# heli-sudoo/HKD-MPC

Measured on NVIDIA B200. Metric: batched HS-DDP solves/sec, higher is better.
Workload: dtype f64

## Files before the change

hkd-mpc_b200/csrc/hsddp_device.cuh:

```cuda
#pragma once
#include <cuda_runtime.h>
#include <stdint.h>
#include <cstddef>
#include "../../include/hsddp_b200.h"
#include "hkd_model.cuh"

#ifdef HSDDP_PROFILE
#define PROF_DECL long long prof_t0_ = clock64();
#define PROF_MARK(sm, slot)                                                         \
    do {                                                                            \
        if (threadIdx.x == 0) {                                                     \
            const long long t1_ = clock64();                                        \
            (sm).profacc[slot] += (unsigned long long)(t1_ - prof_t0_);             \
            prof_t0_ = t1_;                                                         \
        }                                                                           \
    } while (0)
#else
#define PROF_DECL
#define PROF_MARK(sm, slot) do { } while (0)
#endif

namespace hsddp {

constexpr int kThreads = 128;
// ... 30 lines not shown
    unsigned nmask[MAXPH];
    long long ref_off;
    double dt;
    unsigned char ph_of_stage[HSDDP_MAX_STAGES];
    unsigned char ph_of_node[HSDDP_MAX_STAGES + MAXPH];
    unsigned char ss_size[MAXPH];
    unsigned char tdmask[2][MAXPH];
};
static_assert(sizeof(DevSchedule) % 4 == 0, "bind_problem copies the schedule word by word");

struct SolverState {
    double actual_cost, merit, feas, dV_1, dV_2;
    double max_tconstr_prev, max_pconstr_prev, max_tconstr, max_pconstr, merit_rho;
    double reg;
    int rollout_ok, sweep_ok;
};

struct SolveCtl {
    int iter, iter_ou, iter_in, n_sweeps, n_trials, status;
    int active;
    int have_trial;
    int max_al, max_ddp;
    double cost0, feas0;
    double trial_cost, trial_feas;
};

struct BatchPtrs {
    int n_problems, max_stages, max_nodes, _pad;
    const DevSchedule* sched;
    const int* sched_id;
    const double *xr, *ur, *prel, *xinit;
    double* x0;
    double *Xbar, *X, *Xsim_t, *Defect, *dX;
    double *Ubar, *U, *U_t, *dU;
    double* KdX;
    double* K;
    double* lq;
    double* tq;
    double* gcon;
    double* reb;
    double* hcon;
    double* al;
    double* g0h0;
    SolverState* state;
    SolveCtl* ctl;
    const int* active;
    const int* n_active;
    int* next_active;
    int* next_count;
    int* zero_count;
    int sweep_w1_min;
    int lr_external;
    int _pad2;
    double *ls_X, *ls_Defect, *ls_Xsim, *ls_U, *ls_Ut, *ls_gcon, *ls_hcon, *ls_res;
    int* ls_mail;
    const int* order;
    const int* budget;
    hsddp_info* info;
    hsddp_iter_record* trace;
    unsigned long long* counters;
    int* work_counter;
    int* sm_slots;
    hsddp_constraint_params cp;
};

struct Smem;
struct __align__(16) Smem {
    double H[ro(24)], Y[ro(24)];
    double Z[zo(24)];
    double Qux[ro(16) + kQuuPad];
    double Quu[ro(12)];
    double rec[2][LQ_STRIDE];
    double dfc2[2][24];
    double G[24], Gn[24], Qx[24], Qu[24], wu[24], vtmp[24], vtmp2[24];
    double lxxd[24], lxxTd[24], lxxw[12], lxxTw[12];
    double swdt[4];
    double swc[16];
    double red[kThreads];
    DevSchedule sc;
    SolverState st;
    SolveCtl ctl;
    hsddp_constraint_params cp;
    hsddp_options opt;
    double *Xbar, *X, *Xsim_t, *Defect, *dX, *Ubar, *U, *U_t, *dU, *KdX, *K, *lqg, *tq, *gcon, *reb, *hcon, *al, *g0h0;
    const double *xr, *ur, *prel, *xinit, *x0;
    unsigned long long* prof;
    unsigned long long profacc[16];
    int pid;
    int rot;
    int flag;
    int ibuf[4];
    double dbuf[8];
};

static_assert(offsetof(Smem, dfc2) - offsetof(Smem, H) == sizeof(double) * kSweepDoubles, "kSweepDoubles must cover H..rec");
static_assert(32 * 113 <= kSweepDoubles, "LQ staging buffer does not fit");

__device__ __forceinline__ int virtual_tid(const Smem& sm);
__device__ inline void assign_rotation(int* sm_slots, int& rot_out) {
    unsigned smid;
    asm volatile("mov.u32 %0, %%smid;" : "=r"(smid));
    rot_out = atomicAdd(&sm_slots[smid & 255], 1) & 3;
}
__device__ __forceinline__ int virtual_tid(const Smem& sm) { return (int)((threadIdx.x + 32u * (unsigned)sm.rot) & (kThreads - 1)); }

__device__ __forceinline__ double warp_sum(double v) {
// ... 672 lines not shown
```

hkd-mpc_b200/csrc/hsddp_kernels.cu:

```cuda
#include <cuda_runtime.h>
#include <cooperative_groups.h>
#include <cstdio>
#include <cstdlib>
#include <cstring>
#include <string>
#include <vector>
#include <map>
#include <algorithm>
#include "hsddp_device.cuh"
#include "hsddp_sweep.cuh"
#include "hsddp_sweep_w1.cuh"
#include "hsddp_lr_w1.cuh"

#ifndef HSDDP_MIN_BLOCKS
#define HSDDP_MIN_BLOCKS 6
#endif

namespace hsddp {

constexpr int hsddp_batch_max_groups = 16;

__device__ inline void prepare_merit_block(Smem& sm) {
    if (threadIdx.x == 0) {
        SolverState& st = sm.st;
// ... 355 lines not shown
        if (threadIdx.x == 0) for (int i = 0; i < 16; ++i) atomicAdd(&sm.prof[i], sm.profacc[i]);
#endif
    }
}

struct ResumeLists {
    const int* list[hsddp_batch_max_groups];
    const int* count[hsddp_batch_max_groups];
    int n;
};
template <int MINB>
__global__ void __launch_bounds__(kThreads, MINB) k_solve_resume(BatchPtrs bp, hsddp_options opt, ResumeLists rl) {
    __shared__ Smem sm;
    if (threadIdx.x == 0) assign_rotation(bp.sm_slots, sm.rot);
    for (;;) {
        __syncthreads();
        if (threadIdx.x == 0) {
            int q = atomicAdd(bp.work_counter, 1), pid = -1;
            for (int g = 0; g < rl.n; ++g) {
                const int c = *rl.count[g];
                if (q < c) { pid = rl.list[g][q]; break; }
                q -= c;
            }
            sm.ibuf[3] = pid;
        }
        __syncthreads();
        const int pid = sm.ibuf[3];
        if (pid < 0) break;
        bind_problem(sm, bp, pid);
        if (threadIdx.x == 0) sm.opt = opt;
        __syncthreads();
        while (sm.ctl.active) {
            iter_prep_block(sm, bp);
            iter_sweep_block(sm, bp);
            if (!sm.ctl.active) break;
            iter_forward_block(sm, bp);
        }
        solve_finish_block(sm, bp);
        if (threadIdx.x == 0) { bp.state[pid] = sm.st; bp.ctl[pid] = sm.ctl; }
    }
}

enum SolvePhase { PH_BEGIN = 0, PH_PREP, PH_SWEEP, PH_FORWARD };
#ifndef HSDDP_MINB_SWEEP
#define HSDDP_MINB_SWEEP 5
#endif
#ifndef HSDDP_MINB_OTHER
#define HSDDP_MINB_OTHER 6
#endif
template <int PH>
__global__ void __launch_bounds__(kThreads, PH == 2 ? HSDDP_MINB_SWEEP : HSDDP_MINB_OTHER) k_phase(BatchPtrs bp, hsddp_options opt) {
    __shared__ Smem sm;
    if (PH == PH_PREP && bp.zero_count && blockIdx.x == 0 && threadIdx.x == 0) *bp.zero_count = 0;
    if (bp.n_active && (int)blockIdx.x >= *bp.n_active) return;
    if (PH == PH_SWEEP && bp.n_active && bp.sweep_w1_min > 0 && *bp.n_active >= bp.sweep_w1_min) return;
    const int pid = bp.active ? bp.active[blockIdx.x] : (int)blockIdx.x;
    if (threadIdx.x == 0) assign_rotation(bp.sm_slots, sm.rot);
    bind_problem(sm, bp, pid);
    if (threadIdx.x == 0) sm.opt = opt;
    __syncthreads();
#ifdef HSDDP_PROFILE
    if (threadIdx.x == 0) for (int i = 0; i < 16; ++i) sm.profacc[i] = 0;
    __syncthreads();
#endif
    if (PH == PH_BEGIN) solve_begin_block(sm, bp);
    if (PH == PH_PREP) iter_prep_block(sm, bp);
    if (PH == PH_SWEEP) iter_sweep_block(sm, bp);
    if (PH == PH_FORWARD) {
        if (sm.ctl.active) iter_forward_block(sm, bp);
    }
    __syncthreads();
    if (PH == PH_BEGIN || PH == PH_FORWARD) {
        if (sm.ctl.active) {
            if (threadIdx.x == 0) bp.next_active[atomicAdd(bp.next_count, 1)] = pid;
        } else {
            solve_finish_block(sm, bp);
        }
    }
    if (threadIdx.x == 0) { bp.state[pid] = sm.st; bp.ctl[pid] = sm.ctl; }
#ifdef HSDDP_PROFILE
    if (threadIdx.x == 0) for (int i = 0; i < 16; ++i) atomicAdd(&sm.prof[i], sm.profacc[i]);
#endif
}

enum StepOp { OP_RESET = 0, OP_ROLLOUT, OP_COST, OP_LQ, OP_SWEEP, OP_SWEEP_REG, OP_LINEAR, OP_MERIT, OP_FORWARD, OP_NOMINAL, OP_AL, OP_REB };

__global__ void __launch_bounds__(kThreads, HSDDP_MIN_BLOCKS) k_step(BatchPtrs bp, hsddp_options opt, int op, double arg, double* darg, int* ok) {
    __shared__ Smem sm;
    const int pid = blockIdx.x;
    if (threadIdx.x == 0) assign_rotation(bp.sm_slots, sm.rot);
    bind_problem(sm, bp, pid);
    if (threadIdx.x == 0) sm.opt = opt;
    __syncthreads();
    int okv = 1;
    switch (op) {
        case OP_RESET: cold_start_block(sm); break;
        case OP_ROLLOUT: okv = hybrid_rollout_block<false>(sm, arg) ? 1 : 0; break;
        case OP_COST: compute_cost_block(sm); break;
        case OP_LQ: lq_approximation_block(sm); break;
        case OP_SWEEP: okv = backward_sweep_block(sm, arg) ? 1 : 0; break;
        case OP_SWEEP_REG: {
            if (threadIdx.x == 0) sm.st.reg = darg[pid];
            __syncthreads();
            int nsw;
            okv = backward_sweep_regularized_block(sm, nsw) ? 1 : 0;
            if (threadIdx.x == 0) darg[pid] = sm.st.reg;
        } break;
        case OP_LINEAR: linear_rollout_block(sm, arg); break;
        case OP_MERIT: prepare_merit_block(sm); break;
        case OP_FORWARD: {
            const double cost_prev = sm.st.actual_cost, merit_prev = sm.st.merit;
            double eps_acc; int ntr;
            okv = line_search_block<false>(sm, eps_acc, ntr) ? 1 : 0;
            if (!okv) { __syncthreads(); if (threadIdx.x == 0) { sm.st.actual_cost = cost_prev; sm.st.merit = merit_prev; } }
            if (threadIdx.x == 0 && darg) darg[pid] = eps_acc;
        } break;
        case OP_NOMINAL: update_nominal_block(sm); break;
        case OP_AL: update_al_block(sm); break;
        case OP_REB: update_reb_block(sm); break;
        default: break;
    }
    __syncthreads();
    if (threadIdx.x == 0) { bp.state[pid] = sm.st; if (ok) ok[pid] = okv; }
}

__global__ void k_command(BatchPtrs bp, int n_steps, hsddp_mpc_command* out) {
    const int pid = blockIdx.x;
    const DevSchedule& sc = bp.sched[bp.sched_id[pid]];
    hsddp_mpc_command& cmd = out[pid];
    __shared__ int s_stage[HSDDP_CMD_MAX_STEPS], s_node[HSDDP_CMD_MAX_STEPS], s_phase[HSDDP_CMD_MAX_STEPS];
    if (threadIdx.x == 0) {
        int s = 0, i = 0;
        for (int k = 0; k < n_steps; ++k) {
            if (s >= sc.horizon[i]) { s = 0; i++; }
            if (i >= sc.n_phases) { i = sc.n_phases - 1; s = sc.horizon[i] - 1; }
// ... 428 lines not shown
}

}

using namespace hsddp;

static thread_local std::string g_last_error;
const char* hsddp_last_error(void) { return g_last_error.c_str(); }
namespace hsddp { void set_last_error(const std::string& s) { g_last_error = s; } }

#define CK(call)                                                                                   \
    do {                                                                                           \
        cudaError_t e_ = (call);                                                                   \
        if (e_ != cudaSuccess) {                                                                   \
            g_last_error = std::string(#call) + ": " + cudaGetErrorString(e_);                     \
            return HSDDP_ERR_CUDA;                                                                 \
        }                                                                                          \
    } while (0)

struct hsddp_batch {
    int device = 0;
    cudaStream_t stream = nullptr;
    cudaEvent_t ev0 = nullptr, ev1 = nullptr;
    cudaEvent_t slots[8] = {nullptr, nullptr, nullptr, nullptr, nullptr, nullptr, nullptr, nullptr};
    unsigned long long n_solve_launches = 0, n_step_launches = 0;
    int n_sm = 0, blocks_per_sm = 1;
    BatchPtrs bp{};
    std::vector<void*> allocs;
    std::vector<DevSchedule> h_sched;
    std::vector<int> h_sched_id;
    bool has_problems = false;
    bool cold = true;
    float last_ms = 0.f;
    int* d_ok = nullptr;
    double* d_darg = nullptr;
    int solve_mode = 0;
    int* d_active[2] = {nullptr, nullptr};
    int* d_count = nullptr;
    int last_rounds = 0;
    int sweep_kind = 2;
    int w1_min_blocks = 1036;
    bool lr_w1 = true;
    int* d_order = nullptr;
    bool have_order = false, use_order = true;
    bool cluster_ls = true;
    static constexpr int kClusterLsMax = 32;
    static constexpr int kMaxGroups = 16;
    int phased_min_group = 1024;
    int hybrid_rounds = 20, hybrid_groups = 4, hybrid_min_group = 256;
    int phased_groups = 4;
    cudaStream_t gstream[kMaxGroups] = {};
    cudaEvent_t gevent[kMaxGroups] = {};
    cudaEvent_t ev_fork = nullptr;
    hsddp_mpc_command* d_cmd = nullptr;
    bool mpc_ready = false;
    GaitLib lib{};
    int *d_sched_gait = nullptr, *d_sched_window = nullptr, *d_mpc_err = nullptr;
    MpcSched* d_mpc = nullptr;
    float plan = 0.f;
    int node_stride = 0, n_sched = 0;
    bool h_sched_stale = false;
    cudaEvent_t ev_u0 = nullptr, ev_u1 = nullptr;
    int n_gaits = 0;
    std::vector<int> slot_refs;
    std::vector<int> slot_free;
    int* d_restart = nullptr;
    double* d_restart_x0 = nullptr;
    size_t d_restart_cap = 0, d_restart_x0_cap = 0;
    int* d_budget = nullptr;
    long long budget_rounds = -1;
    bool slots_marked = false;
};

namespace {

template <class F>
int guarded(F&& body) {
    try {
        return body();
    } catch (const std::bad_alloc&) {
        g_last_error = "out of host memory";
        return HSDDP_ERR_ARG;
    } catch (const std::exception& e) {
        g_last_error = std::string("unexpected exception: ") + e.what();
        return HSDDP_ERR_STATE;
    } catch (...) {
        g_last_error = "unexpected exception";
        return HSDDP_ERR_STATE;
    }
}

template <class T>
int dalloc(hsddp_batch* b, T** p, size_t n) {
    void* q = nullptr;
    CK(cudaMalloc(&q, n * sizeof(T)));
    b->allocs.push_back(q);
    *p = (T*)q;
    return HSDDP_OK;
}

template <class T>
int scratch(hsddp_batch* b, T** p, size_t* cap, size_t n) {
    if (*cap >= n) return HSDDP_OK;
    void* q = nullptr;
    CK(cudaMalloc(&q, n * sizeof(T)));
    if (*p) {
// ... 48 lines not shown
    else bad = check_budget(opt->max_AL_iter, opt->max_DDP_iter);
    if (bad) { g_last_error = std::string("invalid hsddp_options: ") + bad; return HSDDP_ERR_ARG; }
    return HSDDP_OK;
}

int launch_step(hsddp_batch* b, const hsddp_options* opt, int op, double arg, double* darg_dev, int32_t* ok_host, bool sync = true) {
    if (!b || !b->has_problems) { g_last_error = "no problems set"; return HSDDP_ERR_STATE; }
    int rc = check_opt(opt);
    if (rc) return rc;
    CK(cudaSetDevice(b->device));
    const hsddp_options o = opt ? *opt : default_options();
    k_step<<<b->bp.n_problems, kThreads, 0, b->stream>>>(b->bp, o, op, arg, darg_dev, b->d_ok);
    CK(cudaGetLastError());
    b->n_step_launches++;
    if (ok_host) CK(cudaMemcpyAsync(ok_host, b->d_ok, sizeof(int) * b->bp.n_problems, cudaMemcpyDeviceToHost, b->stream));
    if (sync || ok_host) CK(cudaStreamSynchronize(b->stream));
    if (op != OP_RESET) b->cold = false;
    return HSDDP_OK;
}

}

extern "C" {

static int batch_init(hsddp_batch* b, int device) {
    CK(cudaSetDevice(device));
    b->device = device;
    CK(cudaStreamCreateWithFlags(&b->stream, cudaStreamNonBlocking));
    CK(cudaEventCreate(&b->ev0));
    CK(cudaEventCreate(&b->ev1));
    CK(cudaEventCreate(&b->ev_u0));
    CK(cudaEventCreate(&b->ev_u1));
    for (int i = 0; i < 8; ++i) CK(cudaEventCreate(&b->slots[i]));
    cudaDeviceProp prop;
    CK(cudaGetDeviceProperties(&prop, device));
    b->n_sm = prop.multiProcessorCount;
    CK(cudaOccupancyMaxActiveBlocksPerMultiprocessor(&b->blocks_per_sm, k_solve, kThreads, 0));
    if (b->blocks_per_sm < 1) b->blocks_per_sm = 1;
    if (const char* e = getenv("HSDDP_BLOCKS_PER_SM")) {
        const int v = atoi(e);
        if (v >= 1 && v <= b->blocks_per_sm) b->blocks_per_sm = v;
    }
    CK(cudaEventCreateWithFlags(&b->ev_fork, cudaEventDisableTiming));
    if (const char* e = getenv("HSDDP_PHASED_GROUPS")) {
        const int v = atoi(e);
        if (v >= 1 && v <= hsddp_batch::kMaxGroups) b->phased_groups = v;
    }
    if (const char* e = getenv("HSDDP_PHASED_MIN_GROUP")) { const int v = atoi(e); if (v >= 1) b->phased_min_group = v; }
    if (const char* e = getenv("HSDDP_HYBRID_ROUNDS")) b->hybrid_rounds = atoi(e);
    if (const char* e = getenv("HSDDP_HYBRID_GROUPS")) { const int v = atoi(e); if (v >= 1 && v <= hsddp_batch::kMaxGroups) b->hybrid_groups = v; }
    if (const char* e = getenv("HSDDP_SWEEP_KIND")) b->sweep_kind = atoi(e);
    CK(cudaFuncSetAttribute(k_sweep_w1, cudaFuncAttributePreferredSharedMemoryCarveout, cudaSharedmemCarveoutMaxShared));
    CK(cudaFuncSetAttribute(k_lr_w1, cudaFuncAttributePreferredSharedMemoryCarveout, cudaSharedmemCarveoutMaxShared));
    if (const char* e = getenv("HSDDP_W1_MIN_BLOCKS")) b->w1_min_blocks = atoi(e);
    if (const char* e = getenv("HSDDP_LR_W1")) b->lr_w1 = atoi(e) != 0;
    if (const char* e = getenv("HSDDP_QUEUE_ORDER")) b->use_order = atoi(e) != 0;
    if (const char* e = getenv("HSDDP_CLUSTER_LS")) b->cluster_ls = atoi(e) != 0;
    if (const char* e = getenv("HSDDP_SOLVE_MODE")) {
        const int v = atoi(e);
        if (v >= 0 && v <= 3) b->solve_mode = v;
    }
    return HSDDP_OK;
}

int hsddp_batch_create(int device, hsddp_batch** out) {
    if (!out) return HSDDP_ERR_ARG;
    *out = nullptr;
    int n = 0;
    CK(cudaGetDeviceCount(&n));
    if (device < 0 || device >= n) { g_last_error = "no such CUDA device (this library has no CPU fallback)"; return HSDDP_ERR_CUDA; }
    return guarded([&]() -> int {
        hsddp_batch* b = new hsddp_batch();
        const int rc = batch_init(b, device);
        if (rc != HSDDP_OK) { hsddp_batch_destroy(b); return rc; }
        *out = b;
        return HSDDP_OK;
    });
}

int hsddp_batch_destroy(hsddp_batch* b) {
    if (!b) return HSDDP_OK;
    cudaSetDevice(b->device);
    free_problem_allocs(b);
    if (b->ev0) cudaEventDestroy(b->ev0);
    if (b->ev1) cudaEventDestroy(b->ev1);
    if (b->ev_u0) cudaEventDestroy(b->ev_u0);
    if (b->ev_u1) cudaEventDestroy(b->ev_u1);
    for (int i = 0; i < 8; ++i) if (b->slots[i]) cudaEventDestroy(b->slots[i]);
    if (b->stream) cudaStreamDestroy(b->stream);
    if (b->ev_fork) cudaEventDestroy(b->ev_fork);
    for (int g = 0; g < hsddp_batch::kMaxGroups; ++g) {
        if (b->gevent[g]) cudaEventDestroy(b->gevent[g]);
        if (b->gstream[g]) cudaStreamDestroy(b->gstream[g]);
    }
    delete b;
    return HSDDP_OK;
}

static int alloc_workspace(hsddp_batch* b, int n_problems, int max_stages, int max_nodes) {
    BatchPtrs& bp = b->bp;
    int rc;
    const size_t P = (size_t)n_problems, SN = (size_t)max_nodes * 24, SS = (size_t)max_stages * 24;
    if ((rc = dalloc(b, &bp.x0, P * 24))) return rc;
    if ((rc = dalloc(b, &bp.Xbar, P * SN))) return rc;
    if ((rc = dalloc(b, &bp.X, P * SN))) return rc;
    if ((rc = dalloc(b, &bp.Xsim_t, P * SN))) return rc;
    if ((rc = dalloc(b, &bp.Defect, P * SN))) return rc;
    if ((rc = dalloc(b, &bp.dX, P * SN))) return rc;
    if ((rc = dalloc(b, &bp.Ubar, P * SS))) return rc;
    if ((rc = dalloc(b, &bp.U, P * SS))) return rc;
    if ((rc = dalloc(b, &bp.U_t, P * SS))) return rc;
    if ((rc = dalloc(b, &bp.dU, P * SS))) return rc;
    if ((rc = dalloc(b, &bp.KdX, P * max_stages * 12))) return rc;
    if ((rc = dalloc(b, &bp.K, P * max_stages * 288))) return rc;
    if ((rc = dalloc(b, &bp.lq, P * max_stages * CR_STRIDE))) return rc;
    if ((rc = dalloc(b, &bp.tq, P * MAXPH * TQ_STRIDE))) return rc;
    if ((rc = dalloc(b, &bp.gcon, P * max_stages * 20))) return rc;
    if ((rc = dalloc(b, &bp.reb, P * max_stages * 40))) return rc;
    if ((rc = dalloc(b, &bp.hcon, P * MAXPH * 4))) return rc;
    if ((rc = dalloc(b, &bp.al, P * MAXPH * 16))) return rc;
    if ((rc = dalloc(b, &bp.g0h0, P * 600))) return rc;
    if ((rc = dalloc(b, &bp.state, P))) return rc;
    if ((rc = dalloc(b, &bp.ctl, P))) return rc;
    if ((rc = dalloc(b, &b->d_active[0], P))) return rc;
    if ((rc = dalloc(b, &b->d_active[1], P))) return rc;
    if ((rc = dalloc(b, &b->d_order, P))) return rc;
    if (n_problems <= hsddp_batch::kClusterLsMax) {
        const size_t Q = P * 4;
        if ((rc = dalloc(b, &bp.ls_X, Q * SN)) || (rc = dalloc(b, &bp.ls_Defect, Q * SN)) || (rc = dalloc(b, &bp.ls_Xsim, Q * SN)) ||
            (rc = dalloc(b, &bp.ls_U, Q * SS)) || (rc = dalloc(b, &bp.ls_Ut, Q * SS)) || (rc = dalloc(b, &bp.ls_gcon, Q * max_stages * 20)) ||
            (rc = dalloc(b, &bp.ls_hcon, Q * MAXPH * 4)) || (rc = dalloc(b, &bp.ls_res, Q * 8)) || (rc = dalloc(b, &bp.ls_mail, P)))
            return rc;
        CK(cudaMemset(bp.ls_X, 0, Q * SN * sizeof(double)));
        CK(cudaMemset(bp.ls_Defect, 0, Q * SN * sizeof(double)));
        CK(cudaMemset(bp.ls_Xsim, 0, Q * SN * sizeof(double)));
        CK(cudaMemset(bp.ls_U, 0, Q * SS * sizeof(double)));
        CK(cudaMemset(bp.ls_Ut, 0, Q * SS * sizeof(double)));
        CK(cudaMemset(bp.ls_res, 0, Q * 8 * sizeof(double)));
        CK(cudaMemset(bp.ls_mail, 0, P * sizeof(int)));
    }
    b->have_order = false;
    if ((rc = dalloc(b, &b->d_count, (size_t)2 * hsddp_batch::kMaxGroups))) return rc;
    CK(cudaMemset(bp.ctl, 0, P * sizeof(SolveCtl)));
    if ((rc = dalloc(b, &bp.info, P))) return rc;
    if ((rc = dalloc(b, &bp.trace, P * HSDDP_TRACE_CAP))) return rc;
    if ((rc = dalloc(b, &bp.counters, (size_t)32))) return rc;
    if ((rc = dalloc(b, &bp.work_counter, (size_t)4))) return rc;
    if ((rc = dalloc(b, &bp.sm_slots, (size_t)256))) return rc;
    CK(cudaMemset(bp.sm_slots, 0, 256 * sizeof(int)));
    if ((rc = dalloc(b, &b->d_ok, P))) return rc;
    if ((rc = dalloc(b, &b->d_darg, P))) return rc;
    CK(cudaMemset(bp.x0, 0, P * 24 * sizeof(double)));
    CK(cudaMemset(bp.info, 0, P * sizeof(hsddp_info)));
    CK(cudaMemset(bp.trace, 0, P * HSDDP_TRACE_CAP * sizeof(hsddp_iter_record)));
    CK(cudaMemset(bp.state, 0, P * sizeof(SolverState)));
    CK(cudaMemset(bp.counters, 0, 32 * sizeof(unsigned long long)));
    CK(cudaMemset(bp.tq, 0, P * MAXPH * TQ_STRIDE * sizeof(double)));
    CK(cudaMemset(bp.lq, 0, P * max_stages * CR_STRIDE * sizeof(double)));
    CK(cudaMemset(bp.g0h0, 0, P * 600 * sizeof(double)));
    return HSDDP_OK;
}

int hsddp_batch_set_problems(hsddp_batch* b, int n_schedules, const hsddp_schedule* schedules, int n_problems,
                             const int32_t* schedule_id, const hsddp_constraint_params* cparams) {
    return guarded([&]() -> int {
    if (!b || n_schedules <= 0 || !schedules || n_problems <= 0 || !schedule_id) return HSDDP_ERR_ARG;
    CK(cudaSetDevice(b->device));
    free_problem_allocs(b);
    b->h_sched.assign(n_schedules, DevSchedule{});
    size_t total_nodes = 0;
    int max_stages = 0, max_nodes = 0;
    for (int i = 0; i < n_schedules; ++i) {
        const hsddp_schedule& s = schedules[i];
        if (s.n_phases < 1 || s.n_phases > MAXPH || s.n_stages > HSDDP_MAX_STAGES || !s.xr || !s.ur || !s.prel_r || !s.xinit) {
            g_last_error = "invalid schedule";
            return HSDDP_ERR_ARG;
        }
        DevSchedule& d = b->h_sched[i];
        d.n_phases = s.n_phases; d.n_stages = s.n_stages; d.n_nodes = s.n_nodes; d.dt = s.dt; d.ref_off = (long long)total_nodes;
        int no = 0, so = 0;
        for (int p = 0; p < s.n_phases; ++p) {
            if (s.horizon[p] < 1) { g_last_error = "phase with empty horizon"; return HSDDP_ERR_ARG; }
            d.horizon[p] = s.horizon[p]; d.node_off[p] = no; d.stage_off[p] = so;
            unsigned cm = 0, nm = 0;
            for (int l = 0; l < 4; ++l) { cm |= (s.contact[p][l] ? 1u : 0u) << l; nm |= (s.next_contact[p][l] ? 1u : 0u) << l; }
            d.cmask[p] = cm; d.nmask[p] = nm;
            d.ss_size[p] = (unsigned char)(s.horizon[p] + 1);
            d.tdmask[0][p] = (unsigned char)(~cm & nm & 15u); d.tdmask[1][p] = 0;
            for (int k = 0; k < s.horizon[p] && so + k < HSDDP_MAX_STAGES; ++k) d.ph_of_stage[so + k] = (unsigned char)p;
            for (int k = 0; k <= s.horizon[p] && no + k < HSDDP_MAX_STAGES + MAXPH; ++k) d.ph_of_node[no + k] = (unsigned char)p;
            no += s.horizon[p] + 1; so += s.horizon[p];
        }
        if (no != s.n_nodes || so != s.n_stages) { g_last_error = "schedule node/stage counts inconsistent"; return HSDDP_ERR_ARG; }
        total_nodes += (size_t)s.n_nodes;
        max_stages = std::max(max_stages, s.n_stages);
// ... 324 lines not shown

int hsddp_batch_set_initial_condition(hsddp_batch* b, const double* x0) {
    if (!b || !b->has_problems || !x0) return HSDDP_ERR_ARG;
    CK(cudaSetDevice(b->device));
    CK(cudaMemcpyAsync(b->bp.x0, x0, sizeof(double) * 24 * b->bp.n_problems, cudaMemcpyHostToDevice, b->stream));
    CK(cudaStreamSynchronize(b->stream));
    return HSDDP_OK;
}

int hsddp_batch_reset(hsddp_batch* b) {
    int rc = launch_step(b, nullptr, OP_RESET, 0.0, nullptr, nullptr, false);
    if (rc == HSDDP_OK) b->cold = true;
    return rc;
}

__global__ void k_iota(int* a, int n) {
    const int i = blockIdx.x * blockDim.x + threadIdx.x;
    if (i < n) a[i] = i;
}

__device__ __forceinline__ int order_bin(const hsddp_info& q) {
    const int work = 33 * q.n_iter + 48 * q.n_sweeps + 12 * q.n_trials;
    return 255 - min(max(work >> 6, 0), 255);
}
__global__ void k_order_by_iterations(const hsddp_info* info, int n, int* order) {
    __shared__ int bins[256], start[256];
    for (int i = threadIdx.x; i < 256; i += blockDim.x) bins[i] = 0;
    __syncthreads();
    for (int i = threadIdx.x; i < n; i += blockDim.x) atomicAdd(&bins[order_bin(info[i])], 1);
    __syncthreads();
    if (threadIdx.x == 0) {
        int acc = 0;
        for (int i = 0; i < 256; ++i) { start[i] = acc; acc += bins[i]; }
    }
    __syncthreads();
    for (int bi = threadIdx.x; bi < 256; bi += blockDim.x) {
        if (!bins[bi]) continue;
        int pos = start[bi];
        for (int i = 0; i < n; ++i)
            if (order_bin(info[i]) == bi) order[pos++] = i;
    }
}

static int solve_phased(hsddp_batch* b, const hsddp_options& o, bool hybrid) {
    const int P = b->bp.n_problems;
    int G = hybrid ? b->hybrid_groups : b->phased_groups;
    G = std::min(G, std::max(1, P / (hybrid ? b->hybrid_min_group : b->phased_min_group)));
    G = std::max(1, std::min(G, hsddp_batch::kMaxGroups));
    for (int g = 0; g < G; ++g) {
        if (!b->gstream[g]) {
            CK(cudaStreamCreateWithFlags(&b->gstream[g], cudaStreamNonBlocking));
            CK(cudaEventCreateWithFlags(&b->gevent[g], cudaEventDisableTiming));
        }
    }
    CK(cudaEventRecord(b->ev0, b->stream));
    CK(cudaMemsetAsync(b->d_count, 0, 2 * hsddp_batch::kMaxGroups * sizeof(int), b->stream));
    k_iota<<<(P + 255) / 256, 256, 0, b->stream>>>(b->d_active[0], P);
    CK(cudaEventRecord(b->ev_fork, b->stream));
    const int all_rounds = (int)std::min<long long>(std::max((long long)std::max(0, o.max_AL_iter) * (long long)std::max(0, o.max_DDP_iter), b->budget_rounds), 1000000LL);
    const int rounds = hybrid ? std::min(all_rounds, std::max(0, b->hybrid_rounds)) : all_rounds;
    ResumeLists rl{};
    rl.n = 0;
    const bool use_block = b->sweep_kind != 1, use_w1 = b->sweep_kind != 0;
    int rc = HSDDP_OK;
    for (int g = 0; g < G && rc == HSDDP_OK; ++g) {
        const int lo = (int)((long long)P * g / G), n = (int)((long long)P * (g + 1) / G) - lo;
        if (n <= 0) continue;
        cudaStream_t st = b->gstream[g];
        int* cnt[2] = {b->d_count + 2 * g, b->d_count + 2 * g + 1};
        int* list[2] = {b->d_active[0] + lo, b->d_active[1] + lo};
        if (cudaStreamWaitEvent(st, b->ev_fork, 0) != cudaSuccess) { rc = HSDDP_ERR_CUDA; break; }
        BatchPtrs bp = b->bp;
        bp.sweep_w1_min = b->sweep_kind == 0 ? 0 : b->sweep_kind == 1 ? 1 : b->w1_min_blocks;
        bp.lr_external = (b->lr_w1 && o.MS) ? 1 : 0;
        bp.active = list[0]; bp.n_active = nullptr; bp.next_active = list[1]; bp.next_count = cnt[1]; bp.zero_count = nullptr;
        k_phase<PH_BEGIN><<<n, kThreads, 0, st>>>(bp, o);
        b->n_solve_launches++;
        for (int r = 1; r <= rounds; ++r) {
            const int cur = r & 1;
            bp.active = list[cur]; bp.n_active = cnt[cur]; bp.next_active = list[cur ^ 1]; bp.next_count = cnt[cur ^ 1]; bp.zero_count = cnt[cur ^ 1];
            k_phase<PH_PREP><<<n, kThreads, 0, st>>>(bp, o);
            if (use_block) k_phase<PH_SWEEP><<<n, kThreads, 0, st>>>(bp, o);
            if (use_w1) k_sweep_w1<<<n, 32, 0, st>>>(bp, o);
            if (bp.lr_external) k_lr_w1<<<n, 32, 0, st>>>(bp, o);
            k_phase<PH_FORWARD><<<n, kThreads, 0, st>>>(bp, o);
            b->n_solve_launches += 3 + (use_block && use_w1 ? 1 : 0) + (bp.lr_external ? 1 : 0);
        }
        if (cudaGetLastError() != cudaSuccess) { rc = HSDDP_ERR_CUDA; g_last_error = "kernel launch failed in the phased driver"; }
        const int nxt = (rounds + 1) & 1;
        rl.list[rl.n] = list[nxt]; rl.count[rl.n] = cnt[nxt]; rl.n++;
    }
    b->last_rounds = rounds;
    for (int g = 0; g < G; ++g) {
        if (!b->gstream[g]) continue;
        if (cudaEventRecord(b->gevent[g], b->gstream[g]) == cudaSuccess) cudaStreamWaitEvent(b->stream, b->gevent[g], 0);
    }
    if (hybrid && rounds < all_rounds && rc == HSDDP_OK) {
        CK(cudaMemsetAsync(b->bp.work_counter, 0, sizeof(int), b->stream));
        k_solve_resume<4><<<b->n_sm * 4, kThreads, 0, b->stream>>>(b->bp, o, rl);
        CK(cudaGetLastError());
        b->n_solve_launches++;
    }
    CK(cudaEventRecord(b->ev1, b->stream));
    return rc;
}

int hsddp_batch_set_solve_mode(hsddp_batch* b, int mode) {
    if (!b || mode < 0 || mode > 3) return HSDDP_ERR_ARG;
    b->solve_mode = mode;
    return HSDDP_OK;
}

static int consume_budget(hsddp_batch* b) {
    if (b->budget_rounds < 0) return HSDDP_OK;
    CK(cudaMemsetAsync(b->d_budget, 0xff, sizeof(int) * 2 * b->bp.n_problems, b->stream));
    b->budget_rounds = -1;
    return HSDDP_OK;
}

int hsddp_batch_solve_async(hsddp_batch* b, const hsddp_options* opt) {
    if (!b || !b->has_problems) { g_last_error = "no problems set"; return HSDDP_ERR_STATE; }
    int rc = check_opt(opt);
    if (rc) return rc;
    CK(cudaSetDevice(b->device));
    const hsddp_options o = opt ? *opt : default_options();
    b->cold = false;
    const bool phased = b->solve_mode == 2 || (b->solve_mode == 0 && 2 * b->bp.n_problems >= 11 * b->n_sm * b->blocks_per_sm);
    if (phased || b->solve_mode == 3) {
        rc = solve_phased(b, o, !phased);
        if (rc == HSDDP_OK) rc = consume_budget(b);
        return rc;
    }
    CK(cudaMemsetAsync(b->bp.work_counter, 0, sizeof(int), b->stream));
    CK(cudaEventRecord(b->ev0, b->stream));
    if (b->cluster_ls && b->bp.ls_mail && b->bp.n_problems <= hsddp_batch::kClusterLsMax && o.MS) {
        k_solve_lat4<<<4 * b->bp.n_problems, kThreads, 0, b->stream>>>(b->bp, o);
    } else if (b->bp.n_problems <= 2 * b->n_sm) {
        k_solve_lat<<<b->bp.n_problems, kThreads, 0, b->stream>>>(b->bp, o, 0);
    } else {
// ... 359 lines not shown
```

hkd-mpc_b200/csrc/hsddp_sweep_w1.cuh:

```cuda
#pragma once
#include "hsddp_sweep.cuh"

namespace hsddp {

struct __align__(16) SweepW1 {
    double H[ro(24)], Y[ro(24)];
    double Z[zo(24)];
    double Qux[ro(12) + kQuuPad];
    double Quu[ro(12)];
    double R[hkd::kRSize];
    double cr[CR_STRIDE];
    double dfc[24];
    double zvec[24];
    double G[24], Gn[24], Qx[24], vtmp[24];
    double Qu[12], wu[12];
    double lxxd[24], lxxTd[24], lxxw[12], lxxTw[12];
    double swc[16], swdt[4];
    double sbuf[24];
    double dbuf[4];
    int n_phases, n_stages, verdict, _pad;
    int horizon[MAXPH], node_off[MAXPH], stage_off[MAXPH];
    unsigned cmask[MAXPH], nmask[MAXPH];
};
static_assert(offsetof(SweepW1, Quu) - offsetof(SweepW1, Qux) == sizeof(double) * (ro(12) + kQuuPad), "Qux and Quu must be contiguous");
// ... 480 lines not shown
                    }
                }
            }
            __syncwarp();
            double* W = sm.Qux;
#pragma unroll 1
            for (int pass = 0; pass < 2; ++pass) {
                const double* A = (pass ? P : sm.H) + ro(t) + g;
                const double* B = (pass ? W : P) + ro(t) + g;
                double* Cm = (pass ? sm.H : W) + ro(g) + 2 * t;
                double gacc = 0.0;
                if (!pass && lane < 24) {
#pragma unroll
                    for (int m = 0; m < 24; ++m) gacc = fma(P[ro(m) + lane], sm.G[m], gacc);
                }
#pragma unroll 1
                for (int J = 0; J < 3; ++J) {
                    double b[6];
#pragma unroll
                    for (int kk = 0; kk < 6; ++kk) b[kk] = B[8 * J + 104 * kk];
                    double cc[3][2];
#pragma unroll
                    for (int I = 0; I < 3; ++I) { cc[I][0] = 0.0; cc[I][1] = 0.0; }
#pragma unroll
                    for (int kk = 0; kk < 6; ++kk)
#pragma unroll
                        for (int I = 0; I < 3; ++I) dmma(cc[I], A[8 * I + 104 * kk], b[kk]);
                    if (pass) __syncwarp();
#pragma unroll
                    for (int I = 0; I < 3; ++I) st2(Cm + ro(8 * I) + 8 * J, cc[I][0], cc[I][1]);
                }
                __syncwarp();
                if (!pass && lane < 24) sm.G[lane] = gacc;
            }
            __syncwarp();
        }
        double d1, d2;
        if (!w1_phase_sweep(sm, p, ph, reg, dt, rpos, d1, d2)) { success = false; break; }
        dV1 += d1;
        dV2 += d2;
    }
    if (success) {
        for (int e = lane; e < 576; e += 32) p.g0h0[24 + e] = sm.H[ro(e / 24) + e % 24];
        if (lane < 24) p.g0h0[lane] = sm.G[lane];
    }
    __syncwarp();
    dV1o = dV1; dV2o = dV2;
    return success;
}

#ifndef HSDDP_W1_MINB
#define HSDDP_W1_MINB 8
#endif
__global__ void __launch_bounds__(32, HSDDP_W1_MINB) k_sweep_w1(BatchPtrs bp, hsddp_options opt) {
    __shared__ SweepW1 sm;
    const int lane = threadIdx.x;
    if (bp.n_active && ((int)blockIdx.x >= *bp.n_active || *bp.n_active < bp.sweep_w1_min)) return;
    const int pid = bp.active ? bp.active[blockIdx.x] : (int)blockIdx.x;
    const DevSchedule* sc = bp.sched + bp.sched_id[pid];
    if (lane == 0) { sm.n_phases = sc->n_phases; sm.n_stages = sc->n_stages; }
    if (lane < 24) sm.zvec[lane] = (lane == 11) ? 1.0 : 0.0;
    if (lane < MAXPH) {
        sm.horizon[lane] = sc->horizon[lane]; sm.node_off[lane] = sc->node_off[lane]; sm.stage_off[lane] = sc->stage_off[lane];
        sm.cmask[lane] = sc->cmask[lane]; sm.nmask[lane] = sc->nmask[lane];
    }
    const double dt = sc->dt;
    SweepW1Ptrs p;
    p.lqg = bp.lq + (size_t)pid * bp.max_stages * CR_STRIDE;
    p.tq = bp.tq + (size_t)pid * MAXPH * TQ_STRIDE;
    p.Defect = bp.Defect + (size_t)pid * bp.max_nodes * 24;
    p.K = bp.K + (size_t)pid * bp.max_stages * 288;
    p.dU = bp.dU + (size_t)pid * bp.max_stages * 24;
    p.g0h0 = bp.g0h0 + (size_t)pid * 600;
    int rpos[4];
#pragma unroll
    for (int q = 0; q < 4; ++q) rpos[q] = hkd::cr_dense_pos(min(lane + 32 * q, hkd::kCrNnz - 1));
    SolverState& st = bp.state[pid];
    SolveCtl& ctl = bp.ctl[pid];
    double reg = st.reg;
    __syncwarp();
    bool success = false;
    int nsw = 0;
    double dV1 = 0.0, dV2 = 0.0;
    while (!success) {
        ++nsw;
        success = w1_backward_sweep(sm, p, reg, dt, rpos, dV1, dV2);
        if (success) break;
        reg = fmax(reg * opt.update_regularization, 1e-03);
        if (reg > 1e2) break;
    }
    reg = reg / 20;
    if (reg < 1e-06) reg = 0;
    if (lane == 0) {
        st.reg = reg; st.dV_1 = dV1; st.dV_2 = dV2; st.sweep_ok = success ? 1 : 0;
        ctl.n_sweeps += nsw;
        if (ctl.iter <= HSDDP_TRACE_CAP) {
            hsddp_iter_record& rec = bp.trace[(size_t)pid * HSDDP_TRACE_CAP + ctl.iter - 1];
            rec.n_sweeps = nsw; rec.reg_after = reg;
        }
        if (!success) { ctl.status = HSDDP_STATUS_REG_OVERFLOW; ctl.active = 0; }
    }
}

}
```

Before: 56890.

## Run regularization ladder rungs in parallel across thread-block clusters

Adds cluster kernels (block and warp-level) where each of C cluster blocks tries the backward sweep at a different regularization rung, then they exchange outcomes via distributed shared memory and the lowest successful rung commits its gains. Problems with positive reg (likely to need retries) are marked during prep and routed to the cluster kernel on a forked stream, while the normal sweep kernels skip them. This aims to remove serial retry latency on the critical path at the cost of C-fold redundant sweep work, scratch memory, extra copies of K/dU from scratch, and extra launches and stream synchronization each round.

```diff
diff --git a/hkd-mpc_b200/csrc/hsddp_device.cuh b/hkd-mpc_b200/csrc/hsddp_device.cuh
--- a/hkd-mpc_b200/csrc/hsddp_device.cuh
+++ b/hkd-mpc_b200/csrc/hsddp_device.cuh
@@ -106,6 +106,14 @@
     int sweep_w1_min;
     int lr_external;
     int _pad2;
+    int* cl_list;
+    int* cl_count;
+    unsigned char* cl_mark;
+    double* cl_scratch;
+    int cl_cap;
+    int cl_max_active;
+    int cl_force;
+    int _pad3;
     double *ls_X, *ls_Defect, *ls_Xsim, *ls_U, *ls_Ut, *ls_gcon, *ls_hcon, *ls_res;
     int* ls_mail;
     const int* order;
diff --git a/hkd-mpc_b200/csrc/hsddp_kernels.cu b/hkd-mpc_b200/csrc/hsddp_kernels.cu
--- a/hkd-mpc_b200/csrc/hsddp_kernels.cu
+++ b/hkd-mpc_b200/csrc/hsddp_kernels.cu
@@ -431,9 +431,11 @@
 __global__ void __launch_bounds__(kThreads, PH == 2 ? HSDDP_MINB_SWEEP : HSDDP_MINB_OTHER) k_phase(BatchPtrs bp, hsddp_options opt) {
     __shared__ Smem sm;
     if (PH == PH_PREP && bp.zero_count && blockIdx.x == 0 && threadIdx.x == 0) *bp.zero_count = 0;
+    if (PH == PH_FORWARD && bp.cl_count && blockIdx.x == 0 && threadIdx.x == 0) *bp.cl_count = 0;
     if (bp.n_active && (int)blockIdx.x >= *bp.n_active) return;
     if (PH == PH_SWEEP && bp.n_active && bp.sweep_w1_min > 0 && *bp.n_active >= bp.sweep_w1_min) return;
     const int pid = bp.active ? bp.active[blockIdx.x] : (int)blockIdx.x;
+    if (PH == PH_SWEEP && bp.cl_mark && bp.cl_mark[pid]) return;
     if (threadIdx.x == 0) assign_rotation(bp.sm_slots, sm.rot);
     bind_problem(sm, bp, pid);
     if (threadIdx.x == 0) sm.opt = opt;
@@ -444,6 +446,14 @@
 #endif
     if (PH == PH_BEGIN) solve_begin_block(sm, bp);
     if (PH == PH_PREP) iter_prep_block(sm, bp);
+    if (PH == PH_PREP && bp.cl_list && threadIdx.x == 0) {
+        unsigned char m = 0;
+        if (bp.cl_force || (*bp.n_active <= bp.cl_max_active && sm.st.reg > 0.0)) {
+            const int q = atomicAdd(bp.cl_count, 1);
+            if (q < bp.cl_cap) { bp.cl_list[q] = pid; m = 1; }
+        }
+        bp.cl_mark[pid] = m;
+    }
     if (PH == PH_SWEEP) iter_sweep_block(sm, bp);
     if (PH == PH_FORWARD) {
         if (sm.ctl.active) iter_forward_block(sm, bp);
@@ -460,6 +470,66 @@
 #ifdef HSDDP_PROFILE
     if (threadIdx.x == 0) for (int i = 0; i < 16; ++i) atomicAdd(&sm.prof[i], sm.profacc[i]);
 #endif
+}
+
+template <int C>
+__global__ void __cluster_dims__(C, 1, 1) __launch_bounds__(kThreads, HSDDP_MINB_SWEEP) k_sweep_cl_block(BatchPtrs bp, hsddp_options opt) {
+    __shared__ Smem sm;
+    __shared__ int post;
+    const int q = (int)blockIdx.x / C, r = (int)blockIdx.x % C;
+    if ((bp.sweep_w1_min > 0 && *bp.n_active >= bp.sweep_w1_min) || q >= min(*bp.cl_count, bp.cl_cap)) return;
+    const int pid = bp.cl_list[q];
+    if (threadIdx.x == 0) assign_rotation(bp.sm_slots, sm.rot);
+    bind_problem(sm, bp, pid);
+    double* const K0 = bp.K + (size_t)pid * bp.max_stages * 288;
+    double* const dU0 = bp.dU + (size_t)pid * bp.max_stages * 24;
+    double* const g0 = bp.g0h0 + (size_t)pid * 600;
+    if (threadIdx.x == 0) {
+        sm.opt = opt;
+        if (r > 0) { sm.K = cl_slot(bp, q, r, C); sm.dU = sm.K + (size_t)bp.max_stages * 288; sm.g0h0 = sm.dU + (size_t)bp.max_stages * 24; }
+    }
+    __syncthreads();
+    double regw = sm.st.reg;
+    bool wvalid = true;
+    for (int w = 0;; ++w) {
+        bool valid;
+        const double reg = cl_rung_reg(regw, r, opt.update_regularization, valid);
+        valid = valid && wvalid;
+        const bool ok = valid && backward_sweep_block(sm, reg);
+        bool exhausted;
+        const int win = cl_exchange<C>(&post, valid ? (ok ? 1 : 0) : 2, exhausted);
+        if (win >= 0) {
+            if (r == win) {
+                if (r > 0) {
+                    const int ns = sm.sc.n_stages;
+                    for (int e = threadIdx.x; e < ns * 144; e += kThreads) reinterpret_cast<double2*>(K0)[e] = reinterpret_cast<const double2*>(sm.K)[e];
+                    for (int e = threadIdx.x; e < ns * 12; e += kThreads) reinterpret_cast<double2*>(dU0)[e] = reinterpret_cast<const double2*>(sm.dU)[e];
+                    for (int e = threadIdx.x; e < 300; e += kThreads) reinterpret_cast<double2*>(g0)[e] = reinterpret_cast<const double2*>(sm.g0h0)[e];
+                }
+                if (threadIdx.x == 0) {
+                    double rg = reg / 20;
+                    if (rg < 1e-06) rg = 0;
+                    sm.st.reg = rg;
+                    const int nsw = w * C + win + 1;
+                    sm.ctl.n_sweeps += nsw;
+                    if (sm.ctl.iter <= HSDDP_TRACE_CAP) {
+                        hsddp_iter_record& rec = bp.trace[(size_t)pid * HSDDP_TRACE_CAP + sm.ctl.iter - 1];
+                        rec.n_sweeps = nsw; rec.reg_after = rg;
+                    }
+                    bp.state[pid] = sm.st; bp.ctl[pid] = sm.ctl;
+                }
+            }
+            return;
+        }
+        if (exhausted) {
+            if (r == 0) {
+                iter_sweep_block(sm, bp);
+                if (threadIdx.x == 0) { bp.state[pid] = sm.st; bp.ctl[pid] = sm.ctl; }
+            }
+            return;
+        }
+        regw = cl_rung_reg(regw, C, opt.update_regularization, wvalid);
+    }
 }
 
 enum StepOp { OP_RESET = 0, OP_ROLLOUT, OP_COST, OP_LQ, OP_SWEEP, OP_SWEEP_REG, OP_LINEAR, OP_MERIT, OP_FORWARD, OP_NOMINAL, OP_AL, OP_REB };
@@ -994,6 +1064,17 @@
     cudaStream_t gstream[kMaxGroups] = {};
     cudaEvent_t gevent[kMaxGroups] = {};
     cudaEvent_t ev_fork = nullptr;
+    bool cl_on = true;
+    int cl_size = 4;
+    int cl_slots = 512;
+    int cl_max_active = 1 << 30;
+    bool cl_force = false;
+    int cl_alloc = 0;
+    int* d_cl_list = nullptr;
+    unsigned char* d_cl_mark = nullptr;
+    double* d_cl_scratch = nullptr;
+    cudaStream_t cstream[kMaxGroups] = {};
+    cudaEvent_t cev_fork[kMaxGroups] = {}, cev_join[kMaxGroups] = {};
     hsddp_mpc_command* d_cmd = nullptr;
     bool mpc_ready = false;
     GaitLib lib{};
@@ -1148,10 +1229,17 @@
     if (const char* e = getenv("HSDDP_SWEEP_KIND")) b->sweep_kind = atoi(e);
     CK(cudaFuncSetAttribute(k_sweep_w1, cudaFuncAttributePreferredSharedMemoryCarveout, cudaSharedmemCarveoutMaxShared));
     CK(cudaFuncSetAttribute(k_lr_w1, cudaFuncAttributePreferredSharedMemoryCarveout, cudaSharedmemCarveoutMaxShared));
+    CK(cudaFuncSetAttribute(k_sweep_cl_w1<2>, cudaFuncAttributePreferredSharedMemoryCarveout, cudaSharedmemCarveoutMaxShared));
+    CK(cudaFuncSetAttribute(k_sweep_cl_w1<4>, cudaFuncAttributePreferredSharedMemoryCarveout, cudaSharedmemCarveoutMaxShared));
     if (const char* e = getenv("HSDDP_W1_MIN_BLOCKS")) b->w1_min_blocks = atoi(e);
     if (const char* e = getenv("HSDDP_LR_W1")) b->lr_w1 = atoi(e) != 0;
     if (const char* e = getenv("HSDDP_QUEUE_ORDER")) b->use_order = atoi(e) != 0;
     if (const char* e = getenv("HSDDP_CLUSTER_LS")) b->cluster_ls = atoi(e) != 0;
+    if (const char* e = getenv("HSDDP_CL")) b->cl_on = atoi(e) != 0;
+    if (const char* e = getenv("HSDDP_CL_SIZE")) { const int v = atoi(e); if (v == 2 || v == 4) b->cl_size = v; }
+    if (const char* e = getenv("HSDDP_CL_SLOTS")) { const int v = atoi(e); if (v >= 1) b->cl_slots = v; }
+    if (const char* e = getenv("HSDDP_CL_MAX_ACTIVE")) b->cl_max_active = atoi(e);
+    if (const char* e = getenv("HSDDP_CL_FORCE")) b->cl_force = atoi(e) != 0;
     if (const char* e = getenv("HSDDP_SOLVE_MODE")) {
         const int v = atoi(e);
         if (v >= 0 && v <= 3) b->solve_mode = v;
@@ -1188,6 +1276,9 @@
     for (int g = 0; g < hsddp_batch::kMaxGroups; ++g) {
         if (b->gevent[g]) cudaEventDestroy(b->gevent[g]);
         if (b->gstream[g]) cudaStreamDestroy(b->gstream[g]);
+        if (b->cev_fork[g]) cudaEventDestroy(b->cev_fork[g]);
+        if (b->cev_join[g]) cudaEventDestroy(b->cev_join[g]);
+        if (b->cstream[g]) cudaStreamDestroy(b->cstream[g]);
     }
     delete b;
     return HSDDP_OK;
@@ -1236,7 +1327,14 @@
         CK(cudaMemset(bp.ls_mail, 0, P * sizeof(int)));
     }
     b->have_order = false;
-    if ((rc = dalloc(b, &b->d_count, (size_t)2 * hsddp_batch::kMaxGroups))) return rc;
+    if ((rc = dalloc(b, &b->d_count, (size_t)3 * hsddp_batch::kMaxGroups))) return rc;
+    b->cl_alloc = 0;
+    if (b->cl_on) {
+        b->cl_alloc = std::min(b->cl_slots, n_problems);
+        if ((rc = dalloc(b, &b->d_cl_list, (size_t)b->cl_alloc)) || (rc = dalloc(b, &b->d_cl_mark, P)) ||
+            (rc = dalloc(b, &b->d_cl_scratch, (size_t)b->cl_alloc * (b->cl_size - 1) * ((size_t)max_stages * 312 + 600))))
+            return rc;
+    }
     CK(cudaMemset(bp.ctl, 0, P * sizeof(SolveCtl)));
     if ((rc = dalloc(b, &bp.info, P))) return rc;
     if ((rc = dalloc(b, &bp.trace, P * HSDDP_TRACE_CAP))) return rc;
@@ -1667,9 +1765,14 @@
             CK(cudaStreamCreateWithFlags(&b->gstream[g], cudaStreamNonBlocking));
             CK(cudaEventCreateWithFlags(&b->gevent[g], cudaEventDisableTiming));
         }
+        if (b->cl_alloc && !b->cstream[g]) {
+            CK(cudaStreamCreateWithFlags(&b->cstream[g], cudaStreamNonBlocking));
+            CK(cudaEventCreateWithFlags(&b->cev_fork[g], cudaEventDisableTiming));
+            CK(cudaEventCreateWithFlags(&b->cev_join[g], cudaEventDisableTiming));
+        }
     }
     CK(cudaEventRecord(b->ev0, b->stream));
-    CK(cudaMemsetAsync(b->d_count, 0, 2 * hsddp_batch::kMaxGroups * sizeof(int), b->stream));
+    CK(cudaMemsetAsync(b->d_count, 0, 3 * hsddp_batch::kMaxGroups * sizeof(int), b->stream));
     k_iota<<<(P + 255) / 256, 256, 0, b->stream>>>(b->d_active[0], P);
     CK(cudaEventRecord(b->ev_fork, b->stream));
     const int all_rounds = (int)std::min<long long>(std::max((long long)std::max(0, o.max_AL_iter) * (long long)std::max(0, o.max_DDP_iter), b->budget_rounds), 1000000LL);
@@ -1688,6 +1791,13 @@
         BatchPtrs bp = b->bp;
         bp.sweep_w1_min = b->sweep_kind == 0 ? 0 : b->sweep_kind == 1 ? 1 : b->w1_min_blocks;
         bp.lr_external = (b->lr_w1 && o.MS) ? 1 : 0;
+        const int C = b->cl_size, cap = b->cl_alloc / G;
+        if (cap > 0) {
+            bp.cl_list = b->d_cl_list + cap * g; bp.cl_count = b->d_count + 2 * hsddp_batch::kMaxGroups + g; bp.cl_mark = b->d_cl_mark;
+            bp.cl_scratch = b->d_cl_scratch + (size_t)cap * g * (C - 1) * ((size_t)b->bp.max_stages * 312 + 600);
+            bp.cl_cap = cap; bp.cl_max_active = b->cl_max_active; bp.cl_force = b->cl_force ? 1 : 0;
+        }
+        cudaStream_t cst = b->cstream[g];
         bp.active = list[0]; bp.n_active = nullptr; bp.next_active = list[1]; bp.next_count = cnt[1]; bp.zero_count = nullptr;
         k_phase<PH_BEGIN><<<n, kThreads, 0, st>>>(bp, o);
         b->n_solve_launches++;
@@ -1695,11 +1805,19 @@
             const int cur = r & 1;
             bp.active = list[cur]; bp.n_active = cnt[cur]; bp.next_active = list[cur ^ 1]; bp.next_count = cnt[cur ^ 1]; bp.zero_count = cnt[cur ^ 1];
             k_phase<PH_PREP><<<n, kThreads, 0, st>>>(bp, o);
+            if (cap > 0) {
+                cudaEventRecord(b->cev_fork[g], st);
+                cudaStreamWaitEvent(cst, b->cev_fork[g], 0);
+                if (use_block) { if (C == 4) k_sweep_cl_block<4><<<4 * cap, kThreads, 0, cst>>>(bp, o); else k_sweep_cl_block<2><<<2 * cap, kThreads, 0, cst>>>(bp, o); }
+                if (use_w1) { if (C == 4) k_sweep_cl_w1<4><<<4 * cap, 32, 0, cst>>>(bp, o); else k_sweep_cl_w1<2><<<2 * cap, 32, 0, cst>>>(bp, o); }
+                cudaEventRecord(b->cev_join[g], cst);
+            }
             if (use_block) k_phase<PH_SWEEP><<<n, kThreads, 0, st>>>(bp, o);
             if (use_w1) k_sweep_w1<<<n, 32, 0, st>>>(bp, o);
+            if (cap > 0) cudaStreamWaitEvent(st, b->cev_join[g], 0);
             if (bp.lr_external) k_lr_w1<<<n, 32, 0, st>>>(bp, o);
             k_phase<PH_FORWARD><<<n, kThreads, 0, st>>>(bp, o);
-            b->n_solve_launches += 3 + (use_block && use_w1 ? 1 : 0) + (bp.lr_external ? 1 : 0);
+            b->n_solve_launches += 3 + (use_block && use_w1 ? 1 : 0) + (bp.lr_external ? 1 : 0) + (cap > 0 ? (use_block && use_w1 ? 2 : 1) : 0);
         }
         if (cudaGetLastError() != cudaSuccess) { rc = HSDDP_ERR_CUDA; g_last_error = "kernel launch failed in the phased driver"; }
         const int nxt = (rounds + 1) & 1;
diff --git a/hkd-mpc_b200/csrc/hsddp_sweep_w1.cuh b/hkd-mpc_b200/csrc/hsddp_sweep_w1.cuh
--- a/hkd-mpc_b200/csrc/hsddp_sweep_w1.cuh
+++ b/hkd-mpc_b200/csrc/hsddp_sweep_w1.cuh
@@ -556,11 +556,8 @@
 #ifndef HSDDP_W1_MINB
 #define HSDDP_W1_MINB 8
 #endif
-__global__ void __launch_bounds__(32, HSDDP_W1_MINB) k_sweep_w1(BatchPtrs bp, hsddp_options opt) {
-    __shared__ SweepW1 sm;
+__device__ __forceinline__ double w1_bind(SweepW1& sm, const BatchPtrs& bp, int pid, SweepW1Ptrs& p, int (&rpos)[4]) {
     const int lane = threadIdx.x;
-    if (bp.n_active && ((int)blockIdx.x >= *bp.n_active || *bp.n_active < bp.sweep_w1_min)) return;
-    const int pid = bp.active ? bp.active[blockIdx.x] : (int)blockIdx.x;
     const DevSchedule* sc = bp.sched + bp.sched_id[pid];
     if (lane == 0) { sm.n_phases = sc->n_phases; sm.n_stages = sc->n_stages; }
     if (lane < 24) sm.zvec[lane] = (lane == 11) ? 1.0 : 0.0;
@@ -568,20 +565,34 @@
         sm.horizon[lane] = sc->horizon[lane]; sm.node_off[lane] = sc->node_off[lane]; sm.stage_off[lane] = sc->stage_off[lane];
         sm.cmask[lane] = sc->cmask[lane]; sm.nmask[lane] = sc->nmask[lane];
     }
-    const double dt = sc->dt;
-    SweepW1Ptrs p;
     p.lqg = bp.lq + (size_t)pid * bp.max_stages * CR_STRIDE;
     p.tq = bp.tq + (size_t)pid * MAXPH * TQ_STRIDE;
     p.Defect = bp.Defect + (size_t)pid * bp.max_nodes * 24;
     p.K = bp.K + (size_t)pid * bp.max_stages * 288;
     p.dU = bp.dU + (size_t)pid * bp.max_stages * 24;
     p.g0h0 = bp.g0h0 + (size_t)pid * 600;
-    int rpos[4];
 #pragma unroll
     for (int q = 0; q < 4; ++q) rpos[q] = hkd::cr_dense_pos(min(lane + 32 * q, hkd::kCrNnz - 1));
+    return sc->dt;
+}
+
+__device__ __forceinline__ void w1_sweep_commit(const BatchPtrs& bp, int pid, double reg, bool success, int nsw, double dV1, double dV2) {
     SolverState& st = bp.state[pid];
     SolveCtl& ctl = bp.ctl[pid];
-    double reg = st.reg;
+    reg = reg / 20;
+    if (reg < 1e-06) reg = 0;
+    st.reg = reg; st.dV_1 = dV1; st.dV_2 = dV2; st.sweep_ok = success ? 1 : 0;
+    ctl.n_sweeps += nsw;
+    if (ctl.iter <= HSDDP_TRACE_CAP) {
+        hsddp_iter_record& rec = bp.trace[(size_t)pid * HSDDP_TRACE_CAP + ctl.iter - 1];
+        rec.n_sweeps = nsw; rec.reg_after = reg;
+    }
+    if (!success) { ctl.status = HSDDP_STATUS_REG_OVERFLOW; ctl.active = 0; }
+}
+
+__device__ __forceinline__ void w1_sweep_ladder(SweepW1& sm, const SweepW1Ptrs& p, const BatchPtrs& bp, int pid, const hsddp_options& opt,
+                                                double dt, const int (&rpos)[4]) {
+    double reg = bp.state[pid].reg;
     __syncwarp();
     bool success = false;
     int nsw = 0;
@@ -593,17 +604,94 @@
         reg = fmax(reg * opt.update_regularization, 1e-03);
         if (reg > 1e2) break;
     }
-    reg = reg / 20;
-    if (reg < 1e-06) reg = 0;
-    if (lane == 0) {
-        st.reg = reg; st.dV_1 = dV1; st.dV_2 = dV2; st.sweep_ok = success ? 1 : 0;
-        ctl.n_sweeps += nsw;
-        if (ctl.iter <= HSDDP_TRACE_CAP) {
-            hsddp_iter_record& rec = bp.trace[(size_t)pid * HSDDP_TRACE_CAP + ctl.iter - 1];
-            rec.n_sweeps = nsw; rec.reg_after = reg;
-        }
-        if (!success) { ctl.status = HSDDP_STATUS_REG_OVERFLOW; ctl.active = 0; }
-    }
-}
-
-}
+    if (threadIdx.x == 0) w1_sweep_commit(bp, pid, reg, success, nsw, dV1, dV2);
+}
+
+__global__ void __launch_bounds__(32, HSDDP_W1_MINB) k_sweep_w1(BatchPtrs bp, hsddp_options opt) {
+    __shared__ SweepW1 sm;
+    if (bp.n_active && ((int)blockIdx.x >= *bp.n_active || *bp.n_active < bp.sweep_w1_min)) return;
+    const int pid = bp.active ? bp.active[blockIdx.x] : (int)blockIdx.x;
+    if (bp.cl_mark && bp.cl_mark[pid]) return;
+    SweepW1Ptrs p;
+    int rpos[4];
+    const double dt = w1_bind(sm, bp, pid, p, rpos);
+    w1_sweep_ladder(sm, p, bp, pid, opt, dt, rpos);
+}
+
+__device__ __forceinline__ double cl_rung_reg(double reg, int n, double upd, bool& valid) {
+    valid = true;
+    for (int i = 0; i < n; ++i) {
+        reg = fmax(reg * upd, 1e-03);
+        if (reg > 1e2) { valid = false; break; }
+    }
+    return reg;
+}
+__device__ __forceinline__ double* cl_slot(const BatchPtrs& bp, int q, int r, int C) {
+    return bp.cl_scratch + ((size_t)q * (C - 1) + (r - 1)) * ((size_t)bp.max_stages * 312 + 600);
+}
+template <int C>
+__device__ __forceinline__ int cl_exchange(int* post, int v, bool& exhausted) {
+    namespace cg = cooperative_groups;
+    cg::cluster_group cl = cg::this_cluster();
+    if (threadIdx.x == 0) *post = v;
+    cl.sync();
+    int win = -1;
+    exhausted = false;
+#pragma unroll 1
+    for (int j = 0; j < C; ++j) {
+        const int vj = *cl.map_shared_rank(post, j);
+        if (vj == 1) { win = j; break; }
+        if (vj == 2) { exhausted = true; break; }
+    }
+    cl.sync();
+    return win;
+}
+
+template <int C>
+__global__ void __cluster_dims__(C, 1, 1) __launch_bounds__(32, HSDDP_W1_MINB) k_sweep_cl_w1(BatchPtrs bp, hsddp_options opt) {
+    __shared__ SweepW1 sm;
+    __shared__ int post;
+    const int q = (int)blockIdx.x / C, r = (int)blockIdx.x % C;
+    if (*bp.n_active < bp.sweep_w1_min || bp.sweep_w1_min <= 0 || q >= min(*bp.cl_count, bp.cl_cap)) return;
+    const int pid = bp.cl_list[q];
+    SweepW1Ptrs p;
+    int rpos[4];
+    const double dt = w1_bind(sm, bp, pid, p, rpos);
+    const SweepW1Ptrs prob = p;
+    if (r > 0) { p.K = cl_slot(bp, q, r, C); p.dU = p.K + (size_t)bp.max_stages * 288; p.g0h0 = p.dU + (size_t)bp.max_stages * 24; }
+    double regw = bp.state[pid].reg;
+    bool wvalid = true;
+    __syncwarp();
+    for (int w = 0;; ++w) {
+        bool valid;
+        const double reg = cl_rung_reg(regw, r, opt.update_regularization, valid);
+        valid = valid && wvalid;
+        double dV1 = 0.0, dV2 = 0.0;
+        const bool ok = valid && w1_backward_sweep(sm, p, reg, dt, rpos, dV1, dV2);
+        bool exhausted;
+        const int win = cl_exchange<C>(&post, valid ? (ok ? 1 : 0) : 2, exhausted);
+        if (win >= 0) {
+            if (r == win) {
+                if (r > 0) {
+                    const int ns = sm.n_stages;
+                    const double2* src = reinterpret_cast<const double2*>(p.K);
+                    double2* dK = reinterpret_cast<double2*>(prob.K);
+                    for (int e = threadIdx.x; e < ns * 144; e += 32) dK[e] = src[e];
+                    const double2* su = reinterpret_cast<const double2*>(p.dU);
+                    double2* dU = reinterpret_cast<double2*>(prob.dU);
+                    for (int e = threadIdx.x; e < ns * 12; e += 32) dU[e] = su[e];
+                    for (int e = threadIdx.x; e < 300; e += 32) reinterpret_cast<double2*>(prob.g0h0)[e] = reinterpret_cast<const double2*>(p.g0h0)[e];
+                }
+                if (threadIdx.x == 0) w1_sweep_commit(bp, pid, reg, true, w * C + win + 1, dV1, dV2);
+            }
+            return;
+        }
+        if (exhausted) {
+            if (r == 0) w1_sweep_ladder(sm, prob, bp, pid, opt, dt, rpos);
+            return;
+        }
+        regw = cl_rung_reg(regw, C, opt.update_regularization, wvalid);
+    }
+}
+
+}
```

New measurement: 57950 (median of 6 runs). 1.02x the previous value.
